# Jumpat/SegAnyGAussians

Measured on AMD Instinct MI355X. Metric: train views/sec (fwd+bwd), 1080p, 1M Gaussians, 32-D features, higher is better.
Workload: dtype f32; 1 GPU; BASELINE cfg3: 1000000 Gaussians, 1920x1080, 32-D features, fwd+bwd, 1 view/GPU/step; parallelism=view-sharded x1

## Files before the change

### include/mi_rast.h

```cpp
#ifndef MI_RAST_H
#define MI_RAST_H

#include <stddef.h>
#include <stdint.h>

#ifdef __cplusplus
extern "C" {
#endif

#define MI_RAST_OK 0
#define MI_RAST_ERR_INVALID 1
#define MI_RAST_ERR_NON_RGB 2
#define MI_RAST_ERR_HIP 3
#define MI_RAST_ERR_ALLOC 4

#define MI_RAST_FULL_LISTS 1
#define MI_RAST_NO_CULL 4
#define MI_RAST_FAST_EXP 8
#define MI_RAST_EXACT_EXP 128
#define MI_RAST_VERIFY_LISTS 16
#define MI_RAST_TILE_FWD 32
#define MI_RAST_PREZERO_BWD 64
#define MI_RAST_F32_BLEND 2
#define MI_RAST_EQUAL_RUNS 256
// ... 78 lines not shown
    int longest_run,
    const float* mask, float* out_color, float* out_mask, float* out_depth,
    int flags, void* features_ready_event, float* dL_dcolor_next, void* stream);
int mi_rast_last_longest_run(void);
int mi_rast_features_only_supported(int channels);
int mi_rast_fingerprint(int n, const void* const* ptrs, const size_t* nbytes, uint64_t* out , void* stream);

int mi_rast_mark_visible(int P, const float* means3D, const float* viewmatrix,
                         const float* projmatrix, uint8_t* present, void* stream);

int mi_rast_mask_forward(
    mi_rast_resize_fn geometry_buffer, void* geometry_user,
    mi_rast_resize_fn binning_buffer, void* binning_user,
    mi_rast_resize_fn image_buffer, void* image_user,
    int P, int width, int height,
    const float* means3D, const float* opacities, const float* mask,
    const float* scales, float scale_modifier, const float* rotations, const float* cov3D_precomp,
    const float* viewmatrix, const float* projmatrix,
    float tan_fovx, float tan_fovy, int prefiltered,
    float* out_mask, int* radii, int debug, int flags, void* stream, int* num_rendered );

int mi_rast_mask_backward(
    int P, int R, int width, int height,
    char* geom_buffer, char* binning_buffer, char* img_buffer,
    const float* dL_dout_mask, float* dL_dmask, int debug, int flags, void* stream);


const char* mi_rast_last_error(void);
const char* mi_rast_version(void);
int mi_rast_supported_channels(int* out, int n);
uint32_t mi_rast_get_higher_msb(uint32_t n);
enum { MI_GEOM_DEPTHS = 0, MI_GEOM_MEANS2D, MI_GEOM_CONIC_OPACITY, MI_GEOM_COV3D, MI_GEOM_RGB,
       MI_GEOM_CLAMPED, MI_GEOM_TILES_TOUCHED, MI_GEOM_DEPTH_KEY, MI_GEOM_INDEX_REC,
       MI_GEOM_CULL_COUNTER, MI_GEOM_BAND_BITS, MI_GEOM_BWD_PACK, MI_GEOM_NFIELDS };
enum { MI_IMG_FINAL_T = 0, MI_IMG_N_CONTRIB, MI_IMG_RANGES, MI_IMG_TILE_CONSUMED, MI_IMG_TILE_COUNT,
       MI_IMG_TILE_CURSOR, MI_IMG_NUM_RENDERED, MI_IMG_TILE_NSURV, MI_IMG_NFIELDS };
enum { MI_BIN_ENTRIES = 0, MI_BIN_SCRATCH, MI_BIN_BLEND_LIST, MI_BIN_NFIELDS };
size_t mi_rast_geometry_layout(int P, size_t* offsets );
size_t mi_rast_image_layout(int width, int height, size_t* offsets );
size_t mi_rast_binning_layout(int R, size_t* offsets );

enum { MI_STAGE_PREPROCESS = 0, MI_STAGE_TILE_SCAN, MI_STAGE_EMIT, MI_STAGE_TILE_SORT,
       MI_STAGE_BLEND_FWD, MI_STAGE_BLEND_BWD, MI_STAGE_GEOM_BWD, MI_STAGE_COUNT };
int mi_rast_profile_enable(int on);
int mi_rast_profile_read(float* ms );

#ifdef __cplusplus
}
#endif
#endif
```

### seganygaussians_amd/_lib.py

```python
from __future__ import annotations

import ctypes as C
import os

from .build import LIB_PATH

RESIZE_FN = C.CFUNCTYPE(C.c_void_p, C.c_size_t, C.c_void_p)

MI_GEOM_FIELDS = ["depths", "means2D", "conic_opacity", "cov3D", "rgb", "clamped", "tiles_touched",
                  "depth_key", "index_rec", "cull_counter", "band_bits", "bwd_pack"]
MI_IMG_FIELDS = ["final_T", "n_contrib", "ranges", "tile_consumed", "tile_count", "tile_cursor", "num_rendered", "tile_nsurv"]
MI_BIN_FIELDS = ["entries", "scratch", "blend_list"]
MI_RAST_FULL_LISTS, MI_RAST_F32_BLEND, MI_RAST_NO_CULL, MI_RAST_FAST_EXP, MI_RAST_VERIFY_LISTS, MI_RAST_TILE_FWD = 1, 2, 4, 8, 16, 32
MI_RAST_PREZERO_BWD = 64
MI_RAST_EXACT_EXP = 128
MI_RAST_EQUAL_RUNS = 256
MI_RAST_BWD_FEATURES_ONLY = 512
MI_STAGES = ["preprocess", "tile_scan", "emit", "tile_sort", "blend_fwd", "blend_bwd", "geom_bwd"]

EXPORTS = [
    "mi_rast_forward", "mi_rast_forward_reuse", "mi_rast_last_longest_run", "mi_rast_fingerprint", "mi_rast_features_only_supported", "mi_rast_backward", "mi_rast_mark_visible", "mi_rast_mask_forward",
    "mi_rast_mask_backward", "mi_rast_last_error", "mi_rast_version", "mi_rast_supported_channels",
    "mi_rast_get_higher_msb", "mi_rast_geometry_layout", "mi_rast_image_layout", "mi_rast_binning_layout",
    "mi_rast_profile_enable", "mi_rast_profile_read",
    "mi_knn_smooth_forward", "mi_knn_smooth_backward",
    "mi_knn_workspace_bytes", "mi_knn_build", "mi_knn_query", "mi_knn_mean_dist2",
    "mi_contrastive_forward", "mi_contrastive_backward",
    "mi_contrastive_pack_masks", "mi_contrastive_cover", "mi_contrastive_targets", "mi_contrastive_loss_forward",
    "mi_contrastive_loss_backward",
]
MASK_SCALES_EXPORTS = ["mi_mask_scales_workspace_bytes", "mi_mask_erode", "mi_mask_scales"]
SEGMENT_EXPORTS = ["mi_segment_scores", "mi_segment_select", "mi_segment_assign", "mi_segment_assign_block"]
MI_SEGMENT_IMAGE, MI_SEGMENT_POINTS = 0, 1
PHOTOMETRIC_EXPORTS = ["mi_photo_loss_workspace_bytes", "mi_photo_loss_window", "mi_photo_loss_forward", "mi_photo_loss_backward"]
MI_PHOTO_L1, MI_PHOTO_SSIM = 1, 2
ALL_EXPORTS = EXPORTS + MASK_SCALES_EXPORTS + SEGMENT_EXPORTS + PHOTOMETRIC_EXPORTS
MI_SEGMENT_PRE = {"none": 0, "l2": 1, "eps": 2}

_lib = None


class MiRastError(RuntimeError):
    pass
# ... 141 lines not shown
```

### seganygaussians_amd/csrc/binning.h

```cpp
#pragma once

#include <type_traits>

#include "common.h"
#include "cull.h"

namespace mirast {

__device__ __forceinline__ uint32_t wave_inclusive_scan(uint32_t v, int lane)
{
#pragma unroll
    for (int o = 1; o < 64; o <<= 1) {
        const uint32_t t = __shfl_up(v, o, 64);
        if (lane >= o) v += t;
    }
    return v;
}

template <int CTRL, int ROW_MASK, int BANK_MASK>
__device__ __forceinline__ uint32_t dpp_or_zero(uint32_t v)
{
    return (uint32_t)__builtin_amdgcn_update_dpp(0, (int)v, CTRL, ROW_MASK, BANK_MASK, false);
}
template <bool MAX = false>
// ... 384 lines not shown
    __syncthreads();
    for (int y = wave; y < (int)gy; y += BIN_THREADS / 64) {
        int carry = 0;
        for (int x0 = 0; x0 < (int)gx; x0 += 64) {
            const int x = x0 + lane;
            int v = x < (int)gx ? s_grid[y * stride + x] : 0;
#pragma unroll
            for (int o = 1; o < 64; o <<= 1) {
                const int t = __shfl_up(v, o, 64);
                if (lane >= o) v += t;
            }
            v += carry;
            if (x < (int)gx) s_grid[y * stride + x] = v;
            carry = __shfl(v, 63, 64);
        }
    }
    __syncthreads();
    uint32_t* my_partial = partial + (size_t)slice_row(blockIdx.x, gridDim.x) * (gx * gy_all) + (size_t)gx * by0;
    for (int x = tid; x < (int)gx; x += BIN_THREADS) {
        int run = 0;
        for (int y = 0; y < (int)gy; y++) {
            run += s_grid[y * stride + x];
            s_grid[y * stride + x] = run;
        }
    }
    __syncthreads();
    for (int t = tid; t < (int)(gx * gy); t += BIN_THREADS) my_partial[t] = (uint32_t)s_grid[(t / (int)gx) * stride + (t % (int)gx)];
}

constexpr int BW_WORDS = 64 * 18;
__host__ __device__ constexpr size_t span_lds_bytes(size_t head_words) { return (((head_words + 3) & ~(size_t)3) + 4 + 16 * BW_WORDS) * sizeof(uint32_t); }
constexpr uint32_t SPAN_MAX_HEAD_WORDS = 40 * 1024 - 16 * BW_WORDS - 64;

__device__ __forceinline__ void wave_lds_fence()
{
    __builtin_amdgcn_fence(__ATOMIC_SEQ_CST, "wavefront");
    __builtin_amdgcn_wave_barrier();
}

__device__ __forceinline__ uint32_t wave_owner(uint32_t* scratch , uint32_t excl, uint32_t incl, uint32_t base, int lane)
{
    const uint64_t first = ballot64(excl <= base && base < incl);
    const uint32_t owner0 = (uint32_t)__builtin_ctzll(first | (1ull << 63));
    scratch[lane] = 0u;
    wave_lds_fence();
    if (incl > excl && excl > base && excl - base < 64u) scratch[excl - base] = (uint32_t)lane;
    wave_lds_fence();
    const uint32_t here = scratch[lane];
    wave_lds_fence();
    return max(wave_inclusive_scan_dpp<true>(here), owner0);
}

template <bool EMIT>
__global__ void __launch_bounds__(1024) bin_spans_kernel(int P, const BlendRec* __restrict__ index_rec,
                                                         const uint32_t* __restrict__ depth_key, const unsigned long long* __restrict__ band_bits,
                                                         uint32_t* __restrict__ partial, uint32_t* __restrict__ tile_total, const uint2* __restrict__ ranges,
                                                         uint2* __restrict__ entries, uint32_t gx, uint32_t gy_all,
                                                         uint32_t band_h, uint32_t nbands, const int* __restrict__ r_slots,
                                                         int* __restrict__ host_r)
{
    extern __shared__ uint32_t s_dyn[];
    __shared__ uint32_t s_plan[MAX_BANDS + 1];
    const int tid = threadIdx.x, lane = tid & 63, wave = tid >> 6;
    if (!EMIT && host_r != nullptr && blockIdx.x == 0 && tid < R_SLOTS) host_r[tid * R_SLOT_STRIDE] = r_slots[tid * R_SLOT_STRIDE];
    if (wave == 0) band_plan(r_slots, nbands, gridDim.x, s_plan, lane);
    __syncthreads();
    if (blockIdx.x >= s_plan[nbands]) return;
    uint32_t band = 0;
    while (band + 1u < nbands && s_plan[band + 1u] <= blockIdx.x) band++;
    const uint32_t nsub = s_plan[band + 1u] - s_plan[band], sub = blockIdx.x - s_plan[band];
    const uint32_t by0 = band * band_h, by1 = min(gy_all, by0 + band_h);
    const uint32_t band_bit = 1u << band;
    const uint32_t gy = by1 - by0;
    const int stride = count_grid_stride(gx);
    const int ntiles = (int)(gx * gy);
    const int tile0 = (int)(gx * by0);
    const int head = EMIT ? ((ntiles + 3) & ~3) : (((int)gy * stride + 3) & ~3);
    uint32_t* s_cnt = s_dyn;
    int* s_grid = reinterpret_cast<int*>(s_dyn);
    uint32_t* s_next = s_dyn + head;
    uint32_t* wb = s_dyn + head + 4 + wave * BW_WORDS;
    uint32_t* w_pre = wb;
    uint32_t* w_rect = wb + 64;
    uint32_t* w_key = wb + 128;
    uint32_t* w_own = wb + 192;
    float4* w_c0 = reinterpret_cast<float4*>(wb + 256);
    float4* w_c1 = reinterpret_cast<float4*>(wb + 512);
    uint32_t* w_tpre = wb + 768;
    uint32_t* w_q0 = wb + 832;
    uint32_t* w_q1 = wb + 896;
    uint32_t* w_sx = wb + 960;
    uint32_t* w_id = wb + 1024;
    uint32_t* w_queue = wb + 1088;
    uint32_t* my_partial = partial + (size_t)blockIdx.x * (band_h * gx);
    if (EMIT) {
        for (int t = tid; t < ntiles; t += 1024) s_cnt[t] = ranges[tile0 + t].x + my_partial[t];
    } else {
        for (int c = tid; c < (int)gy * stride; c += 1024) s_grid[c] = 0;
    }
    if (tid == 0) s_next[0] = 0u;
    __syncthreads();
    const uint32_t nchunks_all = ((uint32_t)P + 63u) / 64u;
    const uint32_t mc0 = (uint32_t)(((uint64_t)sub * nchunks_all) / nsub), mc1 = (uint32_t)(((uint64_t)(sub + 1u) * nchunks_all) / nsub);
    constexpr uint32_t UNIT = 32;
    const unsigned long long* my_bits = band_bits + (size_t)band * nchunks_all;
    uint32_t g_unit = 0, g_next;
    unsigned long long word = 0ull, nword;
    uint32_t cnt = 0, incl = 0, total = 0, r0 = 0;
    auto request_unit = [&]() __attribute__((always_inline)) {
        uint32_t u = 0;
        if (lane == 0) u = atomicAdd(s_next, 1u);
        g_next = mc0 + UNIT * (uint32_t)__builtin_amdgcn_readfirstlane(u);
        nword = my_bits[min(g_next + (uint32_t)lane, nchunks_all - 1u)];
    };
    auto next_unit = [&]() __attribute__((always_inline)) {
        g_unit = g_next;
        word = ((uint32_t)lane < UNIT && g_unit + (uint32_t)lane < mc1) ? nword : 0ull;
        request_unit();
        cnt = (uint32_t)__builtin_popcountll(word);
        incl = wave_inclusive_scan_dpp(cnt);
        total = (uint32_t)__builtin_amdgcn_readlane((int)incl, 63);
        r0 = 0;
    };
    auto take_chunk = [&](uint32_t& id) __attribute__((always_inline)) -> bool {
        uint32_t qn = 0;
        while (qn < 64u) {
            if (r0 == total) {
                if (g_next >= mc1) break;
                next_unit();
                continue;
            }
            const uint32_t t = min(64u - qn, total - r0);
            uint32_t rk = incl - cnt;
            if (incl > r0 && rk < r0 + t) {
// ... 3 lines not shown
            r0 += t;
            qn += t;
        }
        if (qn == 0u) return false;
        wave_lds_fence();
        id = (uint32_t)lane < qn ? w_queue[lane] : 0xFFFFFFFFu;
        wave_lds_fence();
        return true;
    };
    request_unit();
    uint32_t nid = 0xFFFFFFFFu;
    bool have = take_chunk(nid);
    BlendRec nrec = index_rec[nid == 0xFFFFFFFFu ? 0u : nid];
    while (have) {
        const uint32_t id = nid;
        const BlendRec rec = nrec;
        nid = 0xFFFFFFFFu;
        have = take_chunk(nid);
        nrec = index_rec[nid == 0xFFFFFFFFu ? 0u : nid];
        uint32_t h = 0;
        if (id != 0xFFFFFFFFu) {
            const int rad = (int)rec.pm;
            uint2 rmin, rmax;
            getRect(rec.xy.x, rec.xy.y, rad, rmin, rmax, gx, gy_all);
            shrink_rect(rec.xy, rec.co, rad, rmin, rmax);
            rmin.y = max(rmin.y, by0);
            rmax.y = min(rmax.y, by1);
            if (rmax.x > rmin.x && rmax.y > rmin.y) {
                h = rmax.y - rmin.y;
                const SpanPre pre = span_prepare(rec.co, rad);
                w_c0[lane] = make_float4(pre.B, pre.rcpA, pre.twotauA, pre.det);
                w_c1[lane] = make_float4(pre.cull ? pre.ey : -1.0f, pre.ystar, rec.xy.x, rec.xy.y);
                w_rect[lane] = rmin.x | (rmax.x << 10) | (rmin.y << 21);
                if (EMIT) {
                    w_key[lane] = rec.id;
                    w_id[lane] = id;
                }
            }
        }
        const uint32_t hincl = wave_inclusive_scan_dpp(h);
        const uint32_t rows_total = (uint32_t)__builtin_amdgcn_readlane((int)hincl, 63);
        w_pre[lane] = hincl;
        wave_lds_fence();
        for (uint32_t w0 = 0; w0 < rows_total; w0 += 64) {
            const uint32_t k = w0 + (uint32_t)lane;
            uint32_t width = 0;
            const uint32_t g = wave_owner(w_own, hincl - h, hincl, w0, lane);
            if (k < rows_total) {
                const uint32_t prev = g == 0u ? 0u : w_pre[g - 1];
                const uint32_t packed = w_rect[g];
                const float4 c0 = w_c0[g], c1 = w_c1[g];
                const uint32_t cx0 = packed & 1023u, cx1 = (packed >> 10) & 2047u, ty = (packed >> 21) + (k - prev);
                SpanPre pre;
                pre.B = c0.x;
                pre.rcpA = c0.y;
                pre.twotauA = c0.z;
                pre.det = c0.w;
                pre.cull = c1.x >= 0.f;
                pre.ey = c1.x;
                pre.ystar = c1.y;
                const float2 xy = make_float2(c1.z, c1.w);
                int lo0, hi0, lo1, hi1;
                band_columns(pre, xy, (float)(ty * TILE_Y), (int)(2u * cx0), (int)(2u * cx1), lo0, hi0);
                band_columns(pre, xy, (float)(ty * TILE_Y + 8u), (int)(2u * cx0), (int)(2u * cx1), lo1, hi1);
                if (hi0 > lo0 || hi1 > lo1) {
                    const int lo = hi0 > lo0 ? (hi1 > lo1 ? min(lo0, lo1) : lo0) : lo1;
                    const int hi = hi0 > lo0 ? (hi1 > lo1 ? max(hi0, hi1) : hi0) : hi1;
                    const uint32_t sx0 = (uint32_t)lo >> 1, sx1 = ((uint32_t)hi + 1u) >> 1;
                    if (EMIT) {
                        width = sx1 - sx0;
                        w_q0[lane] = (uint32_t)lo0 | ((uint32_t)hi0 << 11) | (g << 22);
                        w_q1[lane] = (uint32_t)lo1 | ((uint32_t)hi1 << 11);
                        w_sx[lane] = sx0 | (ty << 10);
                    } else {
                        int* row = s_grid + (ty - by0) * stride;
                        const int a0 = lo0 >> 1, b0 = (hi0 + 1) >> 1, a1 = lo1 >> 1, b1 = (hi1 + 1) >> 1;
                        if (hi0 > lo0 && hi1 > lo1 && (b0 < a1 || b1 < a0)) {
                            atomicAdd(&row[a0], 1);
                            atomicAdd(&row[b0], -1);
                            atomicAdd(&row[a1], 1);
                            atomicAdd(&row[b1], -1);
                        } else {
                            atomicAdd(&row[sx0], 1);
                            atomicAdd(&row[sx1], -1);
                        }
                    }
                }
            }
            if (EMIT) {
                const uint32_t tincl = wave_inclusive_scan_dpp(width);
                const uint32_t tiles_total = (uint32_t)__builtin_amdgcn_readlane((int)tincl, 63);
                w_tpre[lane] = tincl;
                wave_lds_fence();
                for (uint32_t t0 = 0; t0 < tiles_total; t0 += 64) {
                    const uint32_t kk = t0 + (uint32_t)lane;
                    const uint32_t o = wave_owner(w_own, tincl - width, tincl, t0, lane);
                    if (kk < tiles_total) {
                        const uint32_t prevt = o == 0u ? 0u : w_tpre[o - 1];
                        const uint32_t q0 = w_q0[o], q1 = w_q1[o], sx = w_sx[o];
                        const uint32_t tx = (sx & 1023u) + (kk - prevt), ty = sx >> 10;
                        const uint32_t lo0 = q0 & 2047u, n0 = ((q0 >> 11) & 2047u) - lo0, lo1 = q1 & 2047u, n1 = ((q1 >> 11) & 2047u) - lo1;
                        const uint32_t c = 2u * tx;
                        const uint32_t qmask = (uint32_t)(c - lo0 < n0) | ((uint32_t)(c + 1u - lo0 < n0) << 1) |
                                               ((uint32_t)(c - lo1 < n1) << 2) | ((uint32_t)(c + 1u - lo1 < n1) << 3);
                        if (qmask != 0u) {
                            const uint32_t gg = q0 >> 22;
                            const uint32_t slot = atomicAdd(&s_cnt[(ty - by0) * gx + tx], 1u);
                            entries[slot] = make_uint2(w_key[gg], w_id[gg] | (qmask << ID_BITS));
                        }
                    }
                }
                wave_lds_fence();
            }
        }
        wave_lds_fence();
    }
    if (!EMIT) {
        __syncthreads();
        for (int y = wave; y < (int)gy; y += 16) {
            int carry = 0;
            for (int x0 = 0; x0 < (int)gx; x0 += 64) {
                const int x = x0 + lane;
                int v = x < (int)gx ? s_grid[y * stride + x] : 0;
                v = (int)wave_inclusive_scan_dpp((uint32_t)v) + carry;
                if (x < (int)gx) my_partial[y * (int)gx + x] = v != 0 ? atomicAdd(&tile_total[tile0 + y * (int)gx + x], (uint32_t)v) : 0u;
                carry = __builtin_amdgcn_readlane(v, 63);
            }
        }
    }
}

__global__ void __launch_bounds__(1024) scan_partials_kernel(int ntiles, int nwg, uint32_t* __restrict__ partial,
                                                             uint32_t* __restrict__ tile_total)
{
    __shared__ uint32_t s_sum[16][64];
    const int tl = threadIdx.x & 63, g = threadIdx.x >> 6;
    const int t = blockIdx.x * 64 + tl;
    const int wpg = (nwg + 15) / 16;
    const int w0 = g * wpg, w1 = min(nwg, w0 + wpg);
    uint32_t sum = 0;
    if (t < ntiles)
        for (int w = w0; w < w1; w++) sum += partial[(size_t)w * ntiles + t];
    s_sum[g][tl] = sum;
    __syncthreads();
    uint32_t run = 0;
    for (int gg = 0; gg < g; gg++) run += s_sum[gg][tl];
    if (t < ntiles) {
        for (int w = w0; w < w1; w++) {
            const uint32_t c = partial[(size_t)w * ntiles + t];
            partial[(size_t)w * ntiles + t] = run;
            run += c;
// ... 319 lines not shown
```

### seganygaussians_amd/csrc/mi_rast.hip

```cpp
#include "host.h"

#include <algorithm>
#include <atomic>
#include <cstdio>
#include <cstdlib>
#include <cstring>
#include <mutex>
#include <vector>

#include "binning.h"
#include "blend_bwd.h"
#include "blend_bwd_wave.h"
#include "blend_bwd_feat.h"
#include "blend_fwd.h"
#include "blend_fwd_wave.h"
#ifdef MI_RAST_PROFILING
#include "blend_fwd_x3.h"
#endif
#include "common.h"
#include "geometry.h"

using namespace mirast;

namespace {
// ... 100 lines not shown
    vp.focal_y = H / (2.0f * tan_fovy);
    vp.focal_x = W / (2.0f * tan_fovx);
    vp.scale_modifier = scale_modifier;
    vp.W = W;
    vp.H = H;
    vp.grid_x = (W + TILE_X - 1) / TILE_X;
    vp.grid_y = (H + TILE_Y - 1) / TILE_Y;
    return vp;
}
ViewParams make_blend_view(int W, int H)
{
    ViewParams vp;
    std::memset(&vp, 0, sizeof(vp));
    vp.W = W;
    vp.H = H;
    vp.grid_x = (W + TILE_X - 1) / TILE_X;
    vp.grid_y = (H + TILE_Y - 1) / TILE_Y;
    return vp;
}

struct GeomPtrs {
    float* depths;
    float2* means2D;
    float4* conic_opacity;
    float* cov3D;
    float* rgb;
    uint8_t* clamped;
    uint32_t* tiles_touched;
    uint32_t* depth_key;
    BlendRec* index_rec;
    int* cull_counter;
    unsigned long long* band_bits;
    float* bwd_pack;
};
struct ImgPtrs {
    float* final_T;
    uint32_t* n_contrib;
    uint2* ranges;
    uint32_t* tile_consumed;
    uint32_t* tile_count;
    uint32_t* tile_cursor;
    int* num_rendered;
    uint32_t* tile_nsurv;
    uint32_t* run_bounds;
    uint32_t longest_run;
};
struct BinPtrs {
    uint2* entries;
    uint2* scratch;
    uint32_t* blend_list;
};

GeomPtrs geom_from(char* base, int P)
{
    size_t off[MI_GEOM_NFIELDS];
    mi_rast_geometry_layout(P, off);
    GeomPtrs g;
    g.depths = (float*)(base + off[MI_GEOM_DEPTHS]);
    g.means2D = (float2*)(base + off[MI_GEOM_MEANS2D]);
    g.conic_opacity = (float4*)(base + off[MI_GEOM_CONIC_OPACITY]);
    g.cov3D = (float*)(base + off[MI_GEOM_COV3D]);
    g.rgb = (float*)(base + off[MI_GEOM_RGB]);
    g.clamped = (uint8_t*)(base + off[MI_GEOM_CLAMPED]);
    g.tiles_touched = (uint32_t*)(base + off[MI_GEOM_TILES_TOUCHED]);
    g.depth_key = (uint32_t*)(base + off[MI_GEOM_DEPTH_KEY]);
    g.index_rec = (BlendRec*)(base + off[MI_GEOM_INDEX_REC]);
    g.cull_counter = (int*)(base + off[MI_GEOM_CULL_COUNTER]);
    g.band_bits = (unsigned long long*)(base + off[MI_GEOM_BAND_BITS]);
    g.bwd_pack = (float*)(base + off[MI_GEOM_BWD_PACK]);
    return g;
}
ImgPtrs img_from(char* base, int W, int H)
{
    size_t off[MI_IMG_NFIELDS];
    mi_rast_image_layout(W, H, off);
    ImgPtrs m;
    m.final_T = (float*)(base + off[MI_IMG_FINAL_T]);
    m.n_contrib = (uint32_t*)(base + off[MI_IMG_N_CONTRIB]);
    m.ranges = (uint2*)(base + off[MI_IMG_RANGES]);
    m.tile_consumed = (uint32_t*)(base + off[MI_IMG_TILE_CONSUMED]);
    m.tile_count = (uint32_t*)(base + off[MI_IMG_TILE_COUNT]);
    m.tile_cursor = (uint32_t*)(base + off[MI_IMG_TILE_CURSOR]);
    m.num_rendered = (int*)(base + off[MI_IMG_NUM_RENDERED]);
    m.tile_nsurv = (uint32_t*)(base + off[MI_IMG_TILE_NSURV]);
    m.run_bounds = reinterpret_cast<uint32_t*>(m.num_rendered + R_SLOTS * R_SLOT_STRIDE + NR_RUN_BOUNDS);
    m.longest_run = 0;
    return m;
}
BinPtrs bin_from(char* base, int R)
{
    size_t off[MI_BIN_NFIELDS];
    mi_rast_binning_layout(R, off);
    BinPtrs b;
    b.entries = (uint2*)(base + off[MI_BIN_ENTRIES]);
    b.scratch = (uint2*)(base + off[MI_BIN_SCRATCH]);
    b.blend_list = (uint32_t*)(base + off[MI_BIN_BLEND_LIST]);
    return b;
}

std::atomic<bool> g_attr_set[MAX_DEVICES];
std::mutex g_attr_mutex;

// ... 81 lines not shown
    if (!g_attr_set[dev].load(std::memory_order_acquire)) {
        std::lock_guard<std::mutex> lock(g_attr_mutex);
        if (!g_attr_set[dev].load(std::memory_order_relaxed)) {
            const int max_lds = (int)((BIN_MAX_TILES + 11 * 1024 + 16) * sizeof(uint32_t));
            HIP_TRY(hipFuncSetAttribute((const void*)bin_ranks_kernel<false>, hipFuncAttributeMaxDynamicSharedMemorySize, max_lds));
            HIP_TRY(hipFuncSetAttribute((const void*)bin_ranks_kernel<true>, hipFuncAttributeMaxDynamicSharedMemorySize, max_lds));
            HIP_TRY(hipFuncSetAttribute((const void*)bin_count_kernel, hipFuncAttributeMaxDynamicSharedMemorySize, max_lds));
            HIP_TRY(hipFuncSetAttribute((const void*)bin_spans_kernel<false>, hipFuncAttributeMaxDynamicSharedMemorySize, 160 * 1024 - 256));
            HIP_TRY(hipFuncSetAttribute((const void*)bin_spans_kernel<true>, hipFuncAttributeMaxDynamicSharedMemorySize, 160 * 1024 - 256));
            HIP_TRY(hipFuncSetAttribute((const void*)tile_ranges_kernel, hipFuncAttributeMaxDynamicSharedMemorySize,
                                        (BIN_MAX_TILES_TOTAL + 1) * (int)sizeof(uint32_t)));
            g_attr_set[dev].store(true, std::memory_order_release);
        }
    }
    if (!g_host_sync.init()) return fail(MI_RAST_ERR_HIP, "cannot allocate pinned host buffer / event");
    const bool nocull = (flags & MI_RAST_NO_CULL) != 0;
    const bool full = debug != 0 || nocull || (flags & MI_RAST_FULL_LISTS) != 0;
    const int nwg = full ? bin_workgroups(P) : std::min(BIN_LEAN_WG, (int)lean_nbands + (P + 1023) / 1024);
    const size_t band_tiles = (size_t)band_rows * vp.grid_x;
    const size_t bin_lds = ((size_t)((band_tiles + 3) & ~(size_t)3) + 3 * 1024 + 16) * sizeof(uint32_t);
    {
        StageTimer t(stream, MI_STAGE_TILE_SCAN);
        const size_t cnt_lds = (size_t)(band_rows + 1) * count_grid_stride(vp.grid_x) * sizeof(int);
        for (uint32_t b = 0; full && b < nbands; b++) {
            const uint32_t by0 = b * band_rows, by1 = std::min(vp.grid_y, by0 + band_rows);
            if (full)
                hipLaunchKernelGGL(bin_count_kernel, dim3(nwg), dim3(BIN_THREADS), cnt_lds, stream, P, geom.index_rec, geom.depth_key,
                                   img.tile_count, vp.grid_x, vp.grid_y, by0, by1, (const int*)img.num_rendered,
                                   b == 0 ? g_host_sync.pinned_dev : (int*)nullptr);
        }
        if (!full)
            hipLaunchKernelGGL(bin_spans_kernel<false>, dim3(nwg), dim3(1024), span_lds_bytes((size_t)lean_band_h * count_grid_stride(vp.grid_x)),
                               stream, P, geom.index_rec, geom.depth_key, geom.band_bits, img.tile_count, img.tile_cursor, (const uint2*)nullptr, (uint2*)nullptr,
                               vp.grid_x, vp.grid_y, lean_band_h, lean_nbands, (const int*)img.num_rendered, g_host_sync.pinned_dev);
        HIP_TRY(hipEventRecord(g_host_sync.ev, stream));
        if (full)
            hipLaunchKernelGGL(scan_partials_kernel, dim3((ntiles + 63) / 64), dim3(1024), 0, stream, ntiles, nwg,
                               img.tile_count, img.tile_cursor);
        const uint32_t run_cap = !(flags & MI_RAST_EQUAL_RUNS) ? (uint32_t)RUN_MODEL_CAP : 0u;
        const uint32_t run_fix = (uint32_t)RUN_MODEL_FIX;
        hipLaunchKernelGGL(tile_ranges_kernel, dim3(1), dim3(1024),
                           ((size_t)std::min(ntiles, BIN_MAX_TILES_TOTAL) + 1) * sizeof(uint32_t), stream, ntiles, img.tile_cursor,
                           img.ranges, img.num_rendered + R_SLOTS * R_SLOT_STRIDE, (const int*)img.num_rendered,
                           g_host_sync.pinned_dev + R_SLOTS * R_SLOT_STRIDE, img.tile_consumed, img.tile_nsurv, img.run_bounds, run_cap, run_fix);
    }
    STAGE_CHECK("tile scan");
    HIP_TRY(hipEventRecord(g_host_sync.ev2, stream));
    HIP_TRY(hipEventSynchronize(g_host_sync.ev));
    long long Rsum = 0;
    for (int k = 0; k < R_SLOTS; k++) Rsum += g_host_sync.pinned[k * R_SLOT_STRIDE];
    if (Rsum > 0x7fffffffll) return fail(MI_RAST_ERR_INVALID, "more than 2^31 tile overlaps");
    const int R = (int)Rsum;
    *num_rendered = R;

    size_t boff[MI_BIN_NFIELDS];
    const size_t bin_size = mi_rast_binning_layout(R, boff);
    char* bin_base = binning_buffer(bin_size, binning_user);
    if (!bin_base) return fail(MI_RAST_ERR_ALLOC, "binning buffer callback returned NULL");
    bin = bin_from(bin_base, R);
    const bool verify = !full && (flags & MI_RAST_VERIFY_LISTS) != 0;
    if (R > 0) {
        if (verify) HIP_TRY(hipMemsetAsync(bin.entries, 0, (size_t)R * sizeof(uint2), stream));
        {
            StageTimer t(stream, MI_STAGE_EMIT);
            const size_t emit_lds = bin_lds + 8 * 1024 * sizeof(uint32_t);
            for (uint32_t b = 0; full && b < nbands; b++) {
                const uint32_t by0 = b * band_rows, by1 = std::min(vp.grid_y, by0 + band_rows);
                if (nocull)
                    hipLaunchKernelGGL(bin_ranks_kernel<true>, dim3(nwg), dim3(BIN_THREADS), emit_lds, stream, P, geom.index_rec, geom.depth_key,
                                       img.tile_count, img.ranges, bin.entries, vp.grid_x, vp.grid_y, by0, by1);
                else if (full)
                    hipLaunchKernelGGL(bin_ranks_kernel<false>, dim3(nwg), dim3(BIN_THREADS), emit_lds, stream, P, geom.index_rec, geom.depth_key,
                                       img.tile_count, img.ranges, bin.entries, vp.grid_x, vp.grid_y, by0, by1);
            }
            if (!full)
                hipLaunchKernelGGL(bin_spans_kernel<true>, dim3(nwg), dim3(1024), span_lds_bytes((size_t)lean_band_h * vp.grid_x), stream, P,
                                   geom.index_rec, geom.depth_key, geom.band_bits, img.tile_count, img.tile_cursor, img.ranges, bin.entries, vp.grid_x, vp.grid_y,
                                   lean_band_h, lean_nbands, (const int*)img.num_rendered, (int*)nullptr);
        }
        STAGE_CHECK("emit entries");
        if (verify) {
            uint32_t* ctr = reinterpret_cast<uint32_t*>(img.num_rendered + R_SLOTS * R_SLOT_STRIDE + NR_VERIFY);
            HIP_TRY(hipMemsetAsync(ctr, 0, sizeof(uint32_t), stream));
            hipLaunchKernelGGL(verify_entries_kernel, dim3(ntiles), dim3(256), 0, stream, (uint32_t)ntiles, img.ranges, bin.entries, ctr);
            uint32_t unwritten = 0;
            HIP_TRY(hipMemcpyAsync(&unwritten, ctr, sizeof(uint32_t), hipMemcpyDeviceToHost, stream));
            HIP_TRY(hipStreamSynchronize(stream));
            if (unwritten)
                return fail(MI_RAST_ERR_HIP, "internal error: " + std::to_string(unwritten) + " list slots were counted but not emitted "
                                             "(count / emit passes of bin_spans_kernel disagree)");
        }
        const int* key_bits = img.num_rendered + R_SLOTS * R_SLOT_STRIDE + NR_KEY_BITS;
        {
            StageTimer t(stream, MI_STAGE_TILE_SORT);
#define LAUNCH_TILE_SORT(LO, CAP, FB, NT)                                                                                 \
    hipLaunchKernelGGL((tile_sort_kernel<LO, CAP, FB, NT>), dim3(ntiles), dim3(NT), 0, stream, (uint32_t)ntiles, img.ranges,  \
                       bin.entries, bin.scratch, key_bits, bin.blend_list)
            hipLaunchKernelGGL(tile_sort_wave_kernel<0>, dim3((ntiles + 3) / 4), dim3(256), 0, stream, (uint32_t)ntiles, img.ranges,
                               (const uint2*)bin.entries, bin.blend_list);
            HIP_TRY(hipEventSynchronize(g_host_sync.ev2));
            img.longest_run = longest_of(g_host_sync.pinned + R_SLOTS * R_SLOT_STRIDE + NR_RUN_BOUNDS, (uint32_t)ntiles);
            g_last_longest_run[dev] = (int)img.longest_run;
            if (full ? g_host_sync.pinned[R_SLOTS * R_SLOT_STRIDE + NR_TOTAL] != R : g_host_sync.pinned[R_SLOTS * R_SLOT_STRIDE + NR_TOTAL] > R)
                return fail(MI_RAST_ERR_HIP, "internal error: tile counts do not add up to num_rendered");
            const int max_tile_count = g_host_sync.pinned[R_SLOTS * R_SLOT_STRIDE + NR_LONGEST];
            if (max_tile_count > 1024)
                hipLaunchKernelGGL(tile_sort_wave_kernel<1>, dim3((ntiles + 3) / 4), dim3(256), 0, stream, (uint32_t)ntiles, img.ranges,
                                   (const uint2*)bin.entries, bin.blend_list);
            if (max_tile_count > 2048)
                hipLaunchKernelGGL(tile_sort_wave_kernel<2>, dim3((ntiles + 3) / 4), dim3(256), 0, stream, (uint32_t)ntiles, img.ranges,
                                   (const uint2*)bin.entries, bin.blend_list);
// ... 132 lines not shown
        if (k < n) out[k] = c;
    return k;
}

uint32_t mi_rast_get_higher_msb(uint32_t n)
{
    uint32_t msb = sizeof(n) * 4;
    uint32_t step = msb;
    while (step > 1) {
        step /= 2;
        if (n >> msb) msb += step;
        else msb -= step;
    }
    if (n >> msb) msb++;
    return msb;
}

size_t mi_rast_geometry_layout(int P, size_t* off)
{
    const size_t p = P > 0 ? (size_t)P : 1;
    Carver c;
    off[MI_GEOM_DEPTHS] = c.take(p * sizeof(float));
    off[MI_GEOM_MEANS2D] = c.take(p * sizeof(float2));
    off[MI_GEOM_CONIC_OPACITY] = c.take(p * sizeof(float4));
    off[MI_GEOM_COV3D] = c.take(p * 6 * sizeof(float));
    off[MI_GEOM_RGB] = c.take(p * 3 * sizeof(float));
    off[MI_GEOM_CLAMPED] = c.take(p * 3);
    off[MI_GEOM_TILES_TOUCHED] = c.take(p * sizeof(uint32_t));
    off[MI_GEOM_DEPTH_KEY] = c.take(p * sizeof(uint32_t));
    off[MI_GEOM_INDEX_REC] = c.take(p * sizeof(BlendRec));
    off[MI_GEOM_CULL_COUNTER] = c.take(16);
    off[MI_GEOM_BAND_BITS] = c.take((size_t)MAX_BANDS * ((p + 63) / 64) * sizeof(unsigned long long));
    off[MI_GEOM_BWD_PACK] = c.take(bwd_pack_bytes((int)p));
    return c.off;
}
size_t mi_rast_image_layout(int width, int height, size_t* off)
{
    const size_t n = (size_t)width * height > 0 ? (size_t)width * height : 1;
    const size_t tiles = (size_t)((width + TILE_X - 1) / TILE_X) * ((height + TILE_Y - 1) / TILE_Y);
    Carver c;
    off[MI_IMG_FINAL_T] = c.take(n * sizeof(float));
    off[MI_IMG_N_CONTRIB] = c.take(n * sizeof(uint32_t));
    off[MI_IMG_RANGES] = c.take((tiles ? tiles : 1) * sizeof(uint2));
    off[MI_IMG_TILE_CONSUMED] = c.take((tiles ? tiles : 1) * sizeof(uint32_t));
    constexpr int max_slices = BIN_MAX_WG;
    off[MI_IMG_TILE_COUNT] = c.take((size_t)max_slices * (tiles ? tiles : 1) * sizeof(uint32_t));
    off[MI_IMG_TILE_CURSOR] = c.take((tiles ? tiles : 1) * sizeof(uint32_t));
    off[MI_IMG_NUM_RENDERED] = c.take((R_SLOTS * R_SLOT_STRIDE + 16) * sizeof(int));
    off[MI_IMG_TILE_NSURV] = c.take((tiles ? tiles : 1) * sizeof(uint32_t));
    return c.off;
}
size_t mi_rast_binning_layout(int R, size_t* off)
{
    const size_t r = R > 0 ? (size_t)R : 1;
    Carver c;
    off[MI_BIN_BLEND_LIST] = c.take(r * sizeof(uint32_t));
    off[MI_BIN_ENTRIES] = c.take(r * sizeof(uint2));
    off[MI_BIN_SCRATCH] = c.take(r * sizeof(uint2));
    return c.off;
}

#ifdef MI_RAST_PROFILING
int mi_rast_xcd_stamps(unsigned long long* out, int reset)
{
    static std::vector<unsigned long long> h(2 * (size_t)MI_XCD_LOG_WAVES);
    HIP_TRY(hipDeviceSynchronize());
// ... 399 lines not shown
```

### seganygaussians_amd/geometry_cache.py

```python
from __future__ import annotations

import collections
import ctypes as C
import os
import threading
import weakref

import torch

from . import _lib
from ._ffi import check, dev_ptr, stream_ptr

_NOCACHE_FLAGS = _lib.MI_RAST_FULL_LISTS | _lib.MI_RAST_NO_CULL | _lib.MI_RAST_VERIFY_LISTS | _lib.MI_RAST_TILE_FWD | _lib.MI_RAST_F32_BLEND

_R_SUMS_BYTES = 64 * 128
_WORDS_BYTES = 16 * 4


class GeometryCache:

    def __init__(self, max_bytes=64 << 30):
        self.max_bytes = int(max_bytes)
        self.enabled = True
        self.entries = collections.OrderedDict()
# ... 54 lines not shown
            dev_ptr(x, name, dev)
        fps = self.fingerprints([means3D, opacities, scales, rotations, cov3D_precomp, sh if colours_from_sh else None, viewmatrix,
                                 projmatrix, campos], dev)
        return (dev.index, P, H, W, float(tan_fovx), float(tan_fovy), float(scale_modifier), int(degree),
                int(M) if colours_from_sh else -1, int(flags), tuple(fps))

    def lookup(self, key):
        with self.lock:
            e = self.entries.get(key)
            if e is not None:
                self.entries.move_to_end(key)
                self.hits += 1
            else:
                self.misses += 1
            return e

    def insert(self, key, entry):
        with self.lock:
            old = self.entries.pop(key, None)
            if old is not None:
                self.bytes -= old["bytes"]
            self.entries[key] = entry
            self.bytes += entry["bytes"]
            while self.bytes > self.max_bytes and len(self.entries) > 1:
                _, dropped = self.entries.popitem(last=False)
                self.bytes -= dropped["bytes"]

    def capture(self, key, W, H, rendered, radii, geom, binning, img):
        _, ioff = _lib.image_layout(W, H)
        tiles = ((W + 15) // 16) * ((H + 15) // 16)
        w0 = ioff["num_rendered"] + _R_SUMS_BYTES
        words = img[w0:w0 + _WORDS_BYTES].clone()
        n_list = int(words.view(torch.int32)[0].item()) if rendered > 0 else 0
        entry = {"geom": geom, "num_rendered": rendered, "radii": radii.clone(), "img_bytes": int(img.numel()),
                 "blend_list": binning[:max(4 * n_list, 4)].clone(), "ranges": img[ioff["ranges"]:ioff["ranges"] + 8 * tiles].clone(),
                 "words": words, "longest_run": int(_lib.load().mi_rast_last_longest_run()), "epoch": [0]}
        entry["bytes"] = sum(int(entry[k].numel()) * entry[k].element_size() for k in ("geom", "blend_list", "ranges", "words", "radii"))
        self.insert(key, entry)
        return entry


_geometry_cache = None


def enable_geometry_cache(max_bytes=64 << 30):
    global _geometry_cache
    if _geometry_cache is None:
        _geometry_cache = GeometryCache(max_bytes)
    else:
        _geometry_cache.max_bytes = int(max_bytes)
    _geometry_cache.enabled = True
    return _geometry_cache


def disable_geometry_cache(drop=False):
    global _geometry_cache
    if _geometry_cache is not None:
        _geometry_cache.enabled = False
        if drop:
            _geometry_cache = None


def geometry_cache():
    return _geometry_cache


if os.environ.get("MI_RAST_GEOMETRY_CACHE", "") not in ("", "0"):
# ... 6 lines not shown
```

Before: 913.9 views/s.

## Record surviving row items in count pass and replay them in emit pass

New measurement: 885.6 views/s. -3.1%, worse.

```diff
diff --git a/include/mi_rast.h b/include/mi_rast.h
--- a/include/mi_rast.h
+++ b/include/mi_rast.h
@@ -134,7 +134,9 @@
 uint32_t mi_rast_get_higher_msb(uint32_t n);
 enum { MI_GEOM_DEPTHS = 0, MI_GEOM_MEANS2D, MI_GEOM_CONIC_OPACITY, MI_GEOM_COV3D, MI_GEOM_RGB,
        MI_GEOM_CLAMPED, MI_GEOM_TILES_TOUCHED, MI_GEOM_DEPTH_KEY, MI_GEOM_INDEX_REC,
-       MI_GEOM_CULL_COUNTER, MI_GEOM_BAND_BITS, MI_GEOM_BWD_PACK, MI_GEOM_NFIELDS };
+       MI_GEOM_CULL_COUNTER, MI_GEOM_BAND_BITS, MI_GEOM_BWD_PACK,
+       MI_GEOM_ROW_ITEMS ,
+       MI_GEOM_NFIELDS };
 enum { MI_IMG_FINAL_T = 0, MI_IMG_N_CONTRIB, MI_IMG_RANGES, MI_IMG_TILE_CONSUMED, MI_IMG_TILE_COUNT,
        MI_IMG_TILE_CURSOR, MI_IMG_NUM_RENDERED, MI_IMG_TILE_NSURV, MI_IMG_NFIELDS };
 enum { MI_BIN_ENTRIES = 0, MI_BIN_SCRATCH, MI_BIN_BLEND_LIST, MI_BIN_NFIELDS };
diff --git a/seganygaussians_amd/_lib.py b/seganygaussians_amd/_lib.py
--- a/seganygaussians_amd/_lib.py
+++ b/seganygaussians_amd/_lib.py
@@ -8,7 +8,7 @@
 RESIZE_FN = C.CFUNCTYPE(C.c_void_p, C.c_size_t, C.c_void_p)
 
 MI_GEOM_FIELDS = ["depths", "means2D", "conic_opacity", "cov3D", "rgb", "clamped", "tiles_touched",
-                  "depth_key", "index_rec", "cull_counter", "band_bits", "bwd_pack"]
+                  "depth_key", "index_rec", "cull_counter", "band_bits", "bwd_pack", "row_items"]
 MI_IMG_FIELDS = ["final_T", "n_contrib", "ranges", "tile_consumed", "tile_count", "tile_cursor", "num_rendered", "tile_nsurv"]
 MI_BIN_FIELDS = ["entries", "scratch", "blend_list"]
 MI_RAST_FULL_LISTS, MI_RAST_F32_BLEND, MI_RAST_NO_CULL, MI_RAST_FAST_EXP, MI_RAST_VERIFY_LISTS, MI_RAST_TILE_FWD = 1, 2, 4, 8, 16, 32
diff --git a/seganygaussians_amd/csrc/binning.h b/seganygaussians_amd/csrc/binning.h
--- a/seganygaussians_amd/csrc/binning.h
+++ b/seganygaussians_amd/csrc/binning.h
@@ -440,6 +440,41 @@
 __host__ __device__ constexpr size_t span_lds_bytes(size_t head_words) { return (((head_words + 3) & ~(size_t)3) + 4 + 16 * BW_WORDS) * sizeof(uint32_t); }
 constexpr uint32_t SPAN_MAX_HEAD_WORDS = 40 * 1024 - 16 * BW_WORDS - 64;
 
+struct RowItem {
+    uint32_t lo0, hi0, lo1, hi1, ty, id, key;
+};
+__host__ __device__ inline uint4 item_pack(const RowItem& it)
+{
+    uint4 r;
+    r.x = it.lo0 | (it.hi0 << 11) | ((it.ty & 1023u) << 22);
+    r.y = it.lo1 | (it.hi1 << 11) | ((it.ty >> 10) << 22);
+    r.z = it.id;
+    r.w = it.key;
+    return r;
+}
+__host__ __device__ inline RowItem item_unpack(uint4 r)
+{
+    RowItem it;
+    it.lo0 = r.x & 2047u;
+    it.hi0 = (r.x >> 11) & 2047u;
+    it.lo1 = r.y & 2047u;
+    it.hi1 = (r.y >> 11) & 2047u;
+    it.ty = (r.x >> 22) | ((r.y >> 22) << 10);
+    it.id = r.z;
+    it.key = r.w;
+    return it;
+}
+__host__ __device__ inline void item_span(uint32_t lo0, uint32_t hi0, uint32_t lo1, uint32_t hi1, uint32_t& sx0, uint32_t& sx1)
+{
+    const uint32_t lo = hi0 > lo0 ? (hi1 > lo1 ? (lo0 < lo1 ? lo0 : lo1) : lo0) : lo1;
+    const uint32_t hi = hi0 > lo0 ? (hi1 > lo1 ? (hi0 > hi1 ? hi0 : hi1) : hi0) : hi1;
+    sx0 = lo >> 1;
+    sx1 = (hi + 1u) >> 1;
+}
+constexpr int ITEMS_PER_GAUSSIAN = 3;
+constexpr size_t ITEM_HEADER_BYTES = 2 * BIN_LEAN_WG * sizeof(uint32_t);
+__host__ __device__ inline size_t row_items_bytes(size_t P) { return ITEM_HEADER_BYTES + (size_t)ITEMS_PER_GAUSSIAN * P * sizeof(uint4); }
+
 __device__ __forceinline__ void wave_lds_fence()
 {
     __builtin_amdgcn_fence(__ATOMIC_SEQ_CST, "wavefront");
@@ -465,7 +500,9 @@
                                                          uint32_t* __restrict__ partial, uint32_t* __restrict__ tile_total, const uint2* __restrict__ ranges,
                                                          uint2* __restrict__ entries, uint32_t gx, uint32_t gy_all,
                                                          uint32_t band_h, uint32_t nbands, const int* __restrict__ r_slots,
-                                                         int* __restrict__ host_r)
+                                                         int* __restrict__ host_r, uint32_t* __restrict__ item_hdr ,
+                                                         uint4* __restrict__ item_recs ,
+                                                         uint32_t item_cap )
 {
     extern __shared__ uint32_t s_dyn[];
     __shared__ uint32_t s_plan[MAX_BANDS + 1];
@@ -473,7 +510,10 @@
     if (!EMIT && host_r != nullptr && blockIdx.x == 0 && tid < R_SLOTS) host_r[tid * R_SLOT_STRIDE] = r_slots[tid * R_SLOT_STRIDE];
     if (wave == 0) band_plan(r_slots, nbands, gridDim.x, s_plan, lane);
     __syncthreads();
-    if (blockIdx.x >= s_plan[nbands]) return;
+    if (blockIdx.x >= s_plan[nbands]) {
+        if (!EMIT && item_hdr != nullptr && tid == 0) item_hdr[blockIdx.x] = item_hdr[BIN_LEAN_WG + blockIdx.x] = 0u;
+        return;
+    }
     uint32_t band = 0;
     while (band + 1u < nbands && s_plan[band + 1u] <= blockIdx.x) band++;
     const uint32_t nsub = s_plan[band + 1u] - s_plan[band], sub = blockIdx.x - s_plan[band];
@@ -506,8 +546,67 @@
     } else {
         for (int c = tid; c < (int)gy * stride; c += 1024) s_grid[c] = 0;
     }
-    if (tid == 0) s_next[0] = 0u;
-    __syncthreads();
+    if (tid == 0) s_next[0] = s_next[1] = 0u;
+    __syncthreads();
+    const uint32_t my_cap = item_cap / s_plan[nbands];
+    uint4* my_items = item_recs + (size_t)blockIdx.x * my_cap;
+    auto emit_tiles = [&](uint32_t width) __attribute__((always_inline)) {
+        const uint32_t tincl = wave_inclusive_scan_dpp(width);
+        const uint32_t tiles_total = (uint32_t)__builtin_amdgcn_readlane((int)tincl, 63);
+        w_tpre[lane] = tincl;
+        wave_lds_fence();
+        for (uint32_t t0 = 0; t0 < tiles_total; t0 += 64) {
+            const uint32_t kk = t0 + (uint32_t)lane;
+            const uint32_t o = wave_owner(w_own, tincl - width, tincl, t0, lane);
+            if (kk < tiles_total) {
+                const uint32_t prevt = o == 0u ? 0u : w_tpre[o - 1];
+                const uint32_t q0 = w_q0[o], q1 = w_q1[o], sx = w_sx[o];
+                const uint32_t tx = (sx & 1023u) + (kk - prevt), ty = sx >> 10;
+                const uint32_t lo0 = q0 & 2047u, n0 = ((q0 >> 11) & 2047u) - lo0, lo1 = q1 & 2047u, n1 = ((q1 >> 11) & 2047u) - lo1;
+                const uint32_t c = 2u * tx;
+                const uint32_t qmask = (uint32_t)(c - lo0 < n0) | ((uint32_t)(c + 1u - lo0 < n0) << 1) |
+                                       ((uint32_t)(c - lo1 < n1) << 2) | ((uint32_t)(c + 1u - lo1 < n1) << 3);
+                if (qmask != 0u) {
+                    const uint32_t gg = q0 >> 22;
+                    const uint32_t slot = atomicAdd(&s_cnt[(ty - by0) * gx + tx], 1u);
+                    entries[slot] = make_uint2(w_key[gg], w_id[gg] | (qmask << ID_BITS));
+                }
+            }
+        }
+        wave_lds_fence();
+    };
+    if (EMIT && item_recs != nullptr) {
+        const uint32_t n_items = (uint32_t)__builtin_amdgcn_readfirstlane((int)item_hdr[blockIdx.x]);
+        const uint32_t overflow = (uint32_t)__builtin_amdgcn_readfirstlane((int)item_hdr[BIN_LEAN_WG + blockIdx.x]);
+        if (overflow == 0u) {
+            auto take_window = [&]() __attribute__((always_inline)) -> uint32_t {
+                uint32_t u = 0;
+                if (lane == 0) u = atomicAdd(&s_next[1], 64u);
+                return (uint32_t)__builtin_amdgcn_readfirstlane((int)u);
+            };
+            uint32_t w0 = take_window();
+            uint4 nr = my_items[min(w0 + (uint32_t)lane, n_items ? n_items - 1u : 0u)];
+            while (w0 < n_items) {
+                const bool mine = w0 + (uint32_t)lane < n_items;
+                const RowItem it = item_unpack(nr);
+                w0 = take_window();
+                nr = my_items[min(w0 + (uint32_t)lane, n_items - 1u)];
+                uint32_t width = 0;
+                if (mine) {
+                    uint32_t sx0, sx1;
+                    item_span(it.lo0, it.hi0, it.lo1, it.hi1, sx0, sx1);
+                    width = sx1 - sx0;
+                    w_q0[lane] = it.lo0 | (it.hi0 << 11) | ((uint32_t)lane << 22);
+                    w_q1[lane] = it.lo1 | (it.hi1 << 11);
+                    w_sx[lane] = sx0 | (it.ty << 10);
+                    w_key[lane] = it.key;
+                    w_id[lane] = it.id;
+                }
+                emit_tiles(width);
+            }
+            return;
+        }
+    }
     const uint32_t nchunks_all = ((uint32_t)P + 63u) / 64u;
     const uint32_t mc0 = (uint32_t)(((uint64_t)sub * nchunks_all) / nsub), mc1 = (uint32_t)(((uint64_t)(sub + 1u) * nchunks_all) / nsub);
     constexpr uint32_t UNIT = 32;
@@ -577,10 +676,8 @@
                 w_c0[lane] = make_float4(pre.B, pre.rcpA, pre.twotauA, pre.det);
                 w_c1[lane] = make_float4(pre.cull ? pre.ey : -1.0f, pre.ystar, rec.xy.x, rec.xy.y);
                 w_rect[lane] = rmin.x | (rmax.x << 10) | (rmin.y << 21);
-                if (EMIT) {
-                    w_key[lane] = rec.id;
-                    w_id[lane] = id;
-                }
+                w_key[lane] = rec.id;
+                w_id[lane] = id;
             }
         }
         const uint32_t hincl = wave_inclusive_scan_dpp(h);
@@ -590,6 +687,8 @@
         for (uint32_t w0 = 0; w0 < rows_total; w0 += 64) {
             const uint32_t k = w0 + (uint32_t)lane;
             uint32_t width = 0;
+            bool keep = false;
+            uint4 item = make_uint4(0u, 0u, 0u, 0u);
             const uint32_t g = wave_owner(w_own, hincl - h, hincl, w0, lane);
             if (k < rows_total) {
                 const uint32_t prev = g == 0u ? 0u : w_pre[g - 1];
@@ -618,6 +717,8 @@
                         w_q1[lane] = (uint32_t)lo1 | ((uint32_t)hi1 << 11);
                         w_sx[lane] = sx0 | (ty << 10);
                     } else {
+                        keep = true;
+                        item = item_pack(RowItem{(uint32_t)lo0, (uint32_t)hi0, (uint32_t)lo1, (uint32_t)hi1, ty, w_id[g], w_key[g]});
                         int* row = s_grid + (ty - by0) * stride;
                         const int a0 = lo0 >> 1, b0 = (hi0 + 1) >> 1, a1 = lo1 >> 1, b1 = (hi1 + 1) >> 1;
                         if (hi0 > lo0 && hi1 > lo1 && (b0 < a1 || b1 < a0)) {
@@ -633,35 +734,27 @@
                 }
             }
             if (EMIT) {
-                const uint32_t tincl = wave_inclusive_scan_dpp(width);
-                const uint32_t tiles_total = (uint32_t)__builtin_amdgcn_readlane((int)tincl, 63);
-                w_tpre[lane] = tincl;
-                wave_lds_fence();
-                for (uint32_t t0 = 0; t0 < tiles_total; t0 += 64) {
-                    const uint32_t kk = t0 + (uint32_t)lane;
-                    const uint32_t o = wave_owner(w_own, tincl - width, tincl, t0, lane);
-                    if (kk < tiles_total) {
-                        const uint32_t prevt = o == 0u ? 0u : w_tpre[o - 1];
-                        const uint32_t q0 = w_q0[o], q1 = w_q1[o], sx = w_sx[o];
-                        const uint32_t tx = (sx & 1023u) + (kk - prevt), ty = sx >> 10;
-                        const uint32_t lo0 = q0 & 2047u, n0 = ((q0 >> 11) & 2047u) - lo0, lo1 = q1 & 2047u, n1 = ((q1 >> 11) & 2047u) - lo1;
-                        const uint32_t c = 2u * tx;
-                        const uint32_t qmask = (uint32_t)(c - lo0 < n0) | ((uint32_t)(c + 1u - lo0 < n0) << 1) |
-                                               ((uint32_t)(c - lo1 < n1) << 2) | ((uint32_t)(c + 1u - lo1 < n1) << 3);
-                        if (qmask != 0u) {
-                            const uint32_t gg = q0 >> 22;
-                            const uint32_t slot = atomicAdd(&s_cnt[(ty - by0) * gx + tx], 1u);
-                            entries[slot] = make_uint2(w_key[gg], w_id[gg] | (qmask << ID_BITS));
-                        }
-                    }
+                emit_tiles(width);
+            } else if (item_recs != nullptr) {
+                const uint64_t m = ballot64(keep);
+                if (m != 0ull) {
+                    uint32_t base = 0;
+                    if (lane == 0) base = atomicAdd(&s_next[1], (uint32_t)__builtin_popcountll(m));
+                    base = (uint32_t)__builtin_amdgcn_readfirstlane((int)base);
+                    const uint32_t slot = base + __builtin_amdgcn_mbcnt_hi((uint32_t)(m >> 32), __builtin_amdgcn_mbcnt_lo((uint32_t)m, 0u));
+                    if (keep && slot < my_cap) my_items[slot] = item;
                 }
-                wave_lds_fence();
             }
         }
         wave_lds_fence();
     }
     if (!EMIT) {
         __syncthreads();
+        if (tid == 0 && item_hdr != nullptr) {
+            const uint32_t n = s_next[1];
+            item_hdr[blockIdx.x] = n;
+            item_hdr[BIN_LEAN_WG + blockIdx.x] = n > my_cap ? 1u : 0u;
+        }
         for (int y = wave; y < (int)gy; y += 16) {
             int carry = 0;
             for (int x0 = 0; x0 < (int)gx; x0 += 64) {
diff --git a/seganygaussians_amd/csrc/mi_rast.hip b/seganygaussians_amd/csrc/mi_rast.hip
--- a/seganygaussians_amd/csrc/mi_rast.hip
+++ b/seganygaussians_amd/csrc/mi_rast.hip
@@ -156,6 +156,8 @@
     int* cull_counter;
     unsigned long long* band_bits;
     float* bwd_pack;
+    uint32_t* item_hdr;
+    uint4* item_recs;
 };
 struct ImgPtrs {
     float* final_T;
@@ -192,6 +194,8 @@
     g.cull_counter = (int*)(base + off[MI_GEOM_CULL_COUNTER]);
     g.band_bits = (unsigned long long*)(base + off[MI_GEOM_BAND_BITS]);
     g.bwd_pack = (float*)(base + off[MI_GEOM_BWD_PACK]);
+    g.item_hdr = (uint32_t*)(base + off[MI_GEOM_ROW_ITEMS]);
+    g.item_recs = (uint4*)(base + off[MI_GEOM_ROW_ITEMS] + ITEM_HEADER_BYTES);
     return g;
 }
 ImgPtrs img_from(char* base, int W, int H)
@@ -339,7 +343,8 @@
         if (!full)
             hipLaunchKernelGGL(bin_spans_kernel<false>, dim3(nwg), dim3(1024), span_lds_bytes((size_t)lean_band_h * count_grid_stride(vp.grid_x)),
                                stream, P, geom.index_rec, geom.depth_key, geom.band_bits, img.tile_count, img.tile_cursor, (const uint2*)nullptr, (uint2*)nullptr,
-                               vp.grid_x, vp.grid_y, lean_band_h, lean_nbands, (const int*)img.num_rendered, g_host_sync.pinned_dev);
+                               vp.grid_x, vp.grid_y, lean_band_h, lean_nbands, (const int*)img.num_rendered, g_host_sync.pinned_dev,
+                               geom.item_hdr, geom.item_recs, (uint32_t)ITEMS_PER_GAUSSIAN * (uint32_t)P);
         HIP_TRY(hipEventRecord(g_host_sync.ev, stream));
         if (full)
             hipLaunchKernelGGL(scan_partials_kernel, dim3((ntiles + 63) / 64), dim3(1024), 0, stream, ntiles, nwg,
@@ -383,7 +388,8 @@
             if (!full)
                 hipLaunchKernelGGL(bin_spans_kernel<true>, dim3(nwg), dim3(1024), span_lds_bytes((size_t)lean_band_h * vp.grid_x), stream, P,
                                    geom.index_rec, geom.depth_key, geom.band_bits, img.tile_count, img.tile_cursor, img.ranges, bin.entries, vp.grid_x, vp.grid_y,
-                                   lean_band_h, lean_nbands, (const int*)img.num_rendered, (int*)nullptr);
+                                   lean_band_h, lean_nbands, (const int*)img.num_rendered, (int*)nullptr, geom.item_hdr, geom.item_recs,
+                                   (uint32_t)ITEMS_PER_GAUSSIAN * (uint32_t)P);
         }
         STAGE_CHECK("emit entries");
         if (verify) {
@@ -582,6 +588,7 @@
     off[MI_GEOM_CULL_COUNTER] = c.take(16);
     off[MI_GEOM_BAND_BITS] = c.take((size_t)MAX_BANDS * ((p + 63) / 64) * sizeof(unsigned long long));
     off[MI_GEOM_BWD_PACK] = c.take(bwd_pack_bytes((int)p));
+    off[MI_GEOM_ROW_ITEMS] = c.take(row_items_bytes(p));
     return c.off;
 }
 size_t mi_rast_image_layout(int width, int height, size_t* off)
diff --git a/seganygaussians_amd/geometry_cache.py b/seganygaussians_amd/geometry_cache.py
--- a/seganygaussians_amd/geometry_cache.py
+++ b/seganygaussians_amd/geometry_cache.py
@@ -110,7 +110,8 @@
         w0 = ioff["num_rendered"] + _R_SUMS_BYTES
         words = img[w0:w0 + _WORDS_BYTES].clone()
         n_list = int(words.view(torch.int32)[0].item()) if rendered > 0 else 0
-        entry = {"geom": geom, "num_rendered": rendered, "radii": radii.clone(), "img_bytes": int(img.numel()),
+        _, goff = _lib.geometry_layout(radii.numel())
+        entry = {"geom": geom.view(-1)[:goff["row_items"]], "num_rendered": rendered, "radii": radii.clone(), "img_bytes": int(img.numel()),
                  "blend_list": binning[:max(4 * n_list, 4)].clone(), "ranges": img[ioff["ranges"]:ioff["ranges"] + 8 * tiles].clone(),
                  "words": words, "longest_run": int(_lib.load().mi_rast_last_longest_run()), "epoch": [0]}
         entry["bytes"] = sum(int(entry[k].numel()) * entry[k].element_size() for k in ("geom", "blend_list", "ranges", "words", "radii"))
```
